# JasonTStanley/MultiDroneSim

Hardware: NVIDIA B200
Metric: drone-steps/sec (DYN_GND_DRAG_DW + LQR + order-3 CBF-QP, 8 drones/env) (higher is better)
Workload: dtype f32

## Files before the change

include/mds_b200.h:

```cpp
#ifndef MDS_B200_H
#define MDS_B200_H

#ifdef __cplusplus
extern "C" {
#endif

#define MDS_ABI_VERSION 9
#define MDS_MAX_DRONES_PER_ENV 32
#define MDS_MAX_OBSTACLES 8
#define MDS_OBS_DIM 20
#define MDS_REF_DIM 11

#define MDS_OK 0
#define MDS_ERR_ARG (-1)
#define MDS_ERR_LAUNCH (-2)
#define MDS_ERR_UNSUPPORTED (-3)

enum { MDS_DRONE_CF2X = 0, MDS_DRONE_CF2P = 1 };
enum { MDS_PHYSICS_DYN = 0, MDS_PHYSICS_DYN_GND_DRAG_DW = 1 };

enum { MDS_QP_OPTIMAL = 0, MDS_QP_INFEASIBLE = 1, MDS_QP_ITER_CAP = 2 };

enum {
  MDS_CTRL_GEOMETRIC = 0,
// ... 69 lines not shown
  int max_iter;
  int no_state_bounds;
} MdsCbfParams;

typedef struct MdsTrajSpecF32 { int kind, seg_begin, seg_count, pad; float p[8]; } MdsTrajSpecF32;
typedef struct MdsTrajSpecF64 { int kind, seg_begin, seg_count, pad; double p[8]; } MdsTrajSpecF64;
typedef struct MdsTrajSegF32 { int kind; int has_rot; float t_end; float dur; float p[24]; float rot[12]; } MdsTrajSegF32;
typedef struct MdsTrajSegF64 { int kind; int has_rot; double t_end; double dur; double p[24]; double rot[12]; } MdsTrajSegF64;

enum {
  MDS_STAT_DRONE_STEPS = 0, MDS_STAT_SUM_POS_ERR = 1, MDS_STAT_MAX_POS_ERR = 2,
  MDS_STAT_MIN_BARRIER = 3, MDS_STAT_QP_SOLVES = 4, MDS_STAT_QP_ITERS = 5,
  MDS_STAT_QP_INFEASIBLE = 6, MDS_STAT_QP_ITER_CAP = 7, MDS_STAT_COUNT = 8
};

typedef struct MdsRolloutCfg {
  int ctrl;
  int use_cbf;
  int num_obstacles;
  int write_obs_every;
  int stages;
  double obstacles[MDS_MAX_OBSTACLES * 4];
  const void* lqr_gain_planes_dev;
} MdsRolloutCfg;

int mds_abi_version(void);
const char* mds_last_error(void);
int mds_device_info(int* sm_count, int* cc_major, int* cc_minor, int* l2_bytes);

#include <stddef.h>
int mds_device_alloc(size_t bytes, void** out_dev);
int mds_device_free(void* dev);
int mds_copy_to_device(void* dst_dev, const void* src_host, size_t bytes, void* stream);
int mds_copy_to_host(void* dst_host, const void* src_dev, size_t bytes, void* stream);
int mds_stream_synchronize(void* stream);

int mds_physics_step_f32(const MdsDroneParams* prm, MdsState st, const float* action_dev,
                         const float* ext_force_dev, float* obs_dev, int E, int N, void* stream);
int mds_physics_step_f64(const MdsDroneParams* prm, MdsState st, const double* action_dev,
                         const double* ext_force_dev, double* obs_dev, int E, int N, void* stream);
int mds_physics_step_host_f32(const MdsDroneParams* prm, MdsState st, const float* action_host, float* action_dev,
                              float* obs_dev, float* obs_host, int E, int N, void* stream);
int mds_physics_step_host_f64(const MdsDroneParams* prm, MdsState st, const double* action_host, double* action_dev,
                              double* obs_dev, double* obs_host, int E, int N, void* stream);
int mds_obs_from_state_f32(const MdsDroneParams* prm, MdsState st, float* obs_dev, int D, void* stream);
int mds_obs_from_state_f64(const MdsDroneParams* prm, MdsState st, double* obs_dev, int D, void* stream);
// ... 97 lines not shown
```

multidronesim_b200/_lib.py:

```python
from __future__ import annotations

import ctypes as C
import os

_HERE = os.path.dirname(os.path.abspath(__file__))
LIB_PATH = os.environ.get("MDS_B200_LIB") or os.path.join(_HERE, "csrc", "libmds_b200.so")

MAX_DRONES_PER_ENV = 32
MAX_OBSTACLES = 8
OBS_DIM = 20
REF_DIM = 11
STAT_COUNT = 8
STAT_NAMES = ("drone_steps", "sum_pos_err", "max_pos_err", "min_barrier",
              "qp_solves", "qp_iters", "qp_infeasible", "qp_iter_cap")

DRONE_CF2X, DRONE_CF2P = 0, 1
PHYSICS_DYN, PHYSICS_DYN_GND_DRAG_DW = 0, 1
QP_OPTIMAL, QP_INFEASIBLE, QP_ITER_CAP = 0, 1, 2
CTRL_GEOMETRIC, CTRL_LQR_TORQUE, CTRL_LQR_OMEGA, CTRL_LQR_YANK, CTRL_DSLPID = 0, 1, 2, 3, 4
TRAJ_WAIT, TRAJ_CIRCLE, TRAJ_LEMNISCATE, TRAJ_TABLE = 0, 1, 2, 3
SEG_WAIT, SEG_CIRCLE, SEG_LEMNISCATE, SEG_LINE = 0, 1, 2, 3


class MdsError(RuntimeError):
# ... 28 lines not shown

class GeoGains(C.Structure):
    _fields_ = [(n, C.c_double) for n in ("kp", "kv", "kr", "kw", "g_ctrl", "max_tilt")]


class LqrGains(C.Structure):
    _fields_ = [("K", C.c_double * 48), ("dim", C.c_int)]


class CbfParams(C.Structure):
    _fields_ = [("order", C.c_int), ("zscale", C.c_double), ("safety_radius", C.c_double),
                ("kcbf", C.c_double * 3), ("umax", C.c_double * 4), ("fmin", C.c_double),
                ("fmax", C.c_double), ("max_iter", C.c_int), ("no_state_bounds", C.c_int)]


class RlsCfg(C.Structure):
    _fields_ = [("m", C.c_int), ("target", C.c_int), ("predict_from_xtp1", C.c_int), ("normalize_gain", C.c_int),
                ("project", C.c_int), ("drones_per_env", C.c_int), ("dt", C.c_double), ("theta_code", C.c_ubyte * (16 * 12))]


class RolloutCfg(C.Structure):
    _fields_ = [("ctrl", C.c_int), ("use_cbf", C.c_int), ("num_obstacles", C.c_int),
                ("write_obs_every", C.c_int), ("stages", C.c_int), ("obstacles", C.c_double * (MAX_OBSTACLES * 4)),
                ("lqr_gain_planes_dev", C.c_void_p)]


def traj_spec_dtype(real):
    import numpy as np
    return np.dtype([("kind", "i4"), ("seg_begin", "i4"), ("seg_count", "i4"), ("pad", "i4"), ("p", real, (8,))], align=True)


def traj_seg_dtype(real):
    import numpy as np
    return np.dtype([("kind", "i4"), ("has_rot", "i4"), ("t_end", real), ("dur", real),
                     ("p", real, (24,)), ("rot", real, (12,))], align=True)


_P = C.c_void_p
_I = C.c_int
_D = C.c_double
_PRM = C.POINTER(DroneParams)

_SIGS = {
    "mds_physics_step": [_PRM, State, _P, _P, _P, _I, _I, _P],
    "mds_physics_step_host": [_PRM, State, _P, _P, _P, _P, _I, _I, _P],
    "mds_obs_from_state": [_PRM, State, _P, _I, _P],
    "mds_traj_eval": [_P, _P, _D, _P, _I, _P],
# ... 114 lines not shown
```

multidronesim_b200/csrc/mds_kernels.cu:

```cuda
#include <cuda_runtime.h>
#include <stdio.h>
#include <stdlib.h>
#include <string.h>

#include <mutex>

#include "mds_cbf.cuh"
#include "mds_common.cuh"
#include "mds_ctrl.cuh"
#include "mds_physics.cuh"
#include "mds_sysid.cuh"
#include "mds_traj.cuh"

using namespace mds;

static thread_local char g_err[512] = "";
static int fail(int code, const char* fmt, const char* a = "") {
  snprintf(g_err, sizeof(g_err), fmt, a);
  return code;
}
static int check_launch(const char* what) {
  cudaError_t e = cudaGetLastError();
  if (e != cudaSuccess) {
    snprintf(g_err, sizeof(g_err), "%s: %s", what, cudaGetErrorString(e));
// ... 652 lines not shown
    MDS_REQUIRE(!cfg->use_cbf, "rollout: the CBF filter needs an LQR_OMEGA / LQR_YANK nominal controller");
    Dg = to_dev<Real>(*dsl);
  } else {
    MDS_REQUIRE(lqr && lqr_dim_ok(cfg->ctrl, lqr->dim), "rollout: LQR gains missing or of the wrong dimension");
    L = to_dev<Real>(*lqr);
    if (cfg->ctrl != MDS_CTRL_LQR_TORQUE) MDS_REQUIRE(pid.a && pid.b, "rollout: PID state missing");
  }
  if (cfg->use_cbf) {
    int rc = cbf_args_ok(cbf, N, cfg->num_obstacles);
    if (rc) return rc;
    MDS_REQUIRE((cfg->ctrl == MDS_CTRL_LQR_OMEGA && cbf->order == 2) || (cfg->ctrl == MDS_CTRL_LQR_YANK && cbf->order == 3),
                "rollout: CBF order 2 needs LQR_OMEGA, order 3 needs LQR_YANK");
    C = to_dev<Real>(*cbf);
    rc = qp_scratch_for(N, &C.scr);
    if (rc) return rc;
    for (int i = 0; i < cfg->num_obstacles * 4; ++i) R.obstacles[i] = Real(cfg->obstacles[i]);
    R.u0_pre = Real(prm->m * prm->g);
    R.u0_post = cbf->order == 2 ? Real(prm->m * prm->g) : Real(0);
  } else {
    R.n_obs = 0;
  }
  MDS_REQUIRE(!(cfg->write_obs_every > 0) || obs_log, "rollout: obs_log buffer missing");
  MDS_REQUIRE(cfg->write_obs_every <= 32767, "rollout: write_obs_every must be <= 32767");
  const int NP = next_pow2(N), threads = R.use_cbf ? cbf_block_threads<Real>(NP, N, R.n_obs) : MDS_BLOCK, epb = threads / NP;
  const int blocks = (E + epb - 1) / epb;
  size_t smem = R.use_cbf ? cbf_smem_bytes<Real>(threads, NP, N, R.n_obs) : 32;
  cudaStream_t cs = (cudaStream_t)stream;
  const DroneP<Real> Pd = to_dev<Real>(*prm);
  const StateP<Real> Sd = to_dev<Real>(st);
  const PidP<Real> Pi = to_dev<Real>(pid);
  const size_t obs_elems = (size_t)E * N * MDS_OBS_DIM;
  int mode = cfg->stages == 0 ? mds_rollout_plan(E, N) : cfg->stages;
  if (mode == 7 && cfg->stages == 0 && (cfg->ctrl == MDS_CTRL_DSLPID || NP > 32)) mode = 6;
  MDS_REQUIRE(!(mode == 7 && (cfg->ctrl == MDS_CTRL_DSLPID || NP > 32)), "rollout: plan 7 does not take the DSL PID controller");
  auto obs_slot = [&](int j) -> Real* {
    if (R.write_obs_every > 0 && (j % R.write_obs_every) == 0) return obs_log + (size_t)(j / R.write_obs_every - 1) * obs_elems;
    return obs;
  };
  cudaError_t attr_err = cudaSuccess;
  RolloutLaunch<Real> RL{Pd, R, G, L, C, Dg, Ds, Sd, Pi, specs, segs, action, fext, obs, obs_log, stats, E, N, NP, blocks, threads, phys_spec_of(*prm), smem, cs};
  auto keep = [&](cudaError_t e) { if (e != cudaSuccess) attr_err = e; };
  auto launch_loop = [&]() {
    RolloutLaunch<Real> RLL = RL;
    RLL.threads = R.use_cbf ? cbf_block_threads<Real>(NP, N, R.n_obs, loop_block<Real>()) : loop_block<Real>();
    if (const char* force = getenv("MDS_LOOP_THREADS")) { const int t = atoi(force); if (t >= 32 && t <= RLL.threads && t % 32 == 0) RLL.threads = t; }
    if (RLL.threads < NP) RLL.threads = NP;
    const int epb_l = RLL.threads / NP;
    RLL.blocks = (E + epb_l - 1) / epb_l;
    RLL.smem = R.use_cbf ? cbf_smem_bytes<Real>(RLL.threads, NP, N, R.n_obs) : 32;
    const int every = R.write_obs_every;
    int chunk = 16384;
    if (every > 0) chunk = every >= 16384 ? every : (16384 / every) * every;
    for (int k0 = 0; k0 < K; k0 += chunk) {
      RolloutLaunch<Real> part = RLL;
      if (every > 0) part.obs_log = obs_log + (size_t)(k0 / every) * obs_elems;
      keep(launch_loop_kernel<Real>(part, t0 + k0 * prm->dt_ctrl, prm->dt_ctrl, K - k0 < chunk ? K - k0 : chunk));
    }
  };
  cudaError_t queue_err = cudaSuccess;
  auto launch_queue = [&]() {
    RolloutLaunch<Real> RLQ = RL;
    RLQ.threads = R.use_cbf ? cbf_block_threads<Real>(NP, N, R.n_obs, loop_block<Real>()) : loop_block<Real>();
    if (RLQ.threads < 32) RLQ.threads = 32;
// ... 242 lines not shown
```

multidronesim_b200/csrc/mds_rollout.cuh:

```cuda
#pragma once
#include <cuda_runtime.h>
#include "mds_cbf.cuh"
#include "mds_common.cuh"
#include "mds_ctrl.cuh"
#include "mds_physics.cuh"
#include "mds_traj.cuh"

using namespace mds;

#ifndef MDS_BLOCK
#define MDS_BLOCK 256
#endif
#ifndef MDS_CTRL_MINB
#define MDS_CTRL_MINB 4
#endif
#ifndef MDS_LOOP_MINB
#define MDS_LOOP_MINB 2
#endif
#ifndef MDS_LOOP_BLOCK
#define MDS_LOOP_BLOCK 256
#endif
#ifndef MDS_LOOP_BLOCK_F64
#define MDS_LOOP_BLOCK_F64 192
#endif
// ... 428 lines not shown
  Real obstacles[MDS_MAX_OBSTACLES * 4];
  const Real* lqr_planes;
  int lqr_D;
};

MDS_DEV void atomic_min_double(double* addr, double v) {
  v += 0.0;
  if (v >= 0.0) atomicMin(reinterpret_cast<long long*>(addr), __double_as_longlong(v));
  else atomicMax(reinterpret_cast<unsigned long long*>(addr), (unsigned long long)__double_as_longlong(v));
}
MDS_DEV void atomic_max_double(double* addr, double v) {
  v += 0.0;
  if (v >= 0.0) atomicMax(reinterpret_cast<long long*>(addr), __double_as_longlong(v));
  else atomicMin(reinterpret_cast<unsigned long long*>(addr), (unsigned long long)__double_as_longlong(v));
}

MDS_DEV void prefetch_l1(const void* p) { asm volatile("prefetch.global.L1 [%0];" ::"l"(p)); }

struct StepStats {
  float err, min_h;
  int qp_solves, qp_iters, qp_infeas, qp_cap;
};

template <typename Real, int CTRL, bool USE_CBF, bool PDK = false, int SPEC = 0, int NT = 0>
MDS_DEV void ctrl_body(const DroneP<Real>& P, const RolloutP<Real>& Rc, const GeoP<Real>& G, const LqrP<Real>& L, const CbfP<Real>& C,
                       const DslP<Real>& Dg, const DslStateP<Real>& dst, const CbfSmem<Real>& S, const PidP<Real>& pid,
                       const typename TrajSpecT<Real>::spec& spec,
                       const typename TrajSpecT<Real>::seg* __restrict__ segs, const Obs<Real>& o, const GroupMap& g, int N, int NP,
                       double t, Real rpm[4], StepStats& ss, int pid_idx, M3<Real>* R_out = nullptr) {
  constexpr bool HAS_PID = (CTRL == MDS_CTRL_LQR_OMEGA || CTRL == MDS_CTRL_LQR_YANK);
  constexpr int ORD = CTRL == MDS_CTRL_LQR_OMEGA ? 2 : 3;
  Real u[4] = {Real(0), Real(0), Real(0), Real(0)};
  Ref<Real> ref;
  if (g.valid) {
    ref = eval_traj<Real>(spec, segs, t);
    ss.err = (float)norm(o.p - ref.p);
    if (CTRL == MDS_CTRL_GEOMETRIC) {
      geometric_input(P, G, o, ref, u);
      input_to_action<SPEC>(P, u, rpm);
    } else if (CTRL == MDS_CTRL_DSLPID) {
      DslState<Real> ds = load_dsl(dst, g.d);
      V3<Real> pe;
      dslpid_control(P, Dg, ds, o, ref.p, v3(Real(0), Real(0), ref.yaw), ref.v, v3(Real(0), Real(0), ref.yaw_rate), rpm, &pe);
      store_dsl(dst, g.d, ds);
    } else {
      if (PDK) dlqr_input(P, Rc.lqr_planes, (size_t)Rc.lqr_D, (size_t)g.d, CTRL, o, ref, u);
      else lqr_input(P, L, CTRL, o, ref, u);
      if (CTRL == MDS_CTRL_LQR_TORQUE) input_to_action<SPEC>(P, u, rpm);
    }
  }
  if (HAS_PID) {
    if (USE_CBF) {
      CbfAgent<Real> ag;
      ag.p = {Real(0), Real(0), Real(0)}; ag.dv = ag.p; ag.da = ag.p;
      Real F = Real(0), unom[4] = {Real(0), Real(0), Real(0), Real(0)}, usafe[4] = {Real(0), Real(0), Real(0), Real(0)};
      if (g.valid) {
        if (CTRL == MDS_CTRL_LQR_OMEGA) u[0] = cap_thrust(P, u[0]);
        Real xd[10];
// ... 129 lines not shown
  __shared__ typename Vec4T<Real>::type sm_pos[MDS_BLOCK];
  const int N = ct_n<NT>(N_rt), NP = ct_np<NT>(NP_rt);
  CbfSmem<Real> S = cbf_smem_carve<Real>(smem_raw, NP, N, Rc.n_obs);
  GroupMap g = group_map(N, NP, E);
  StepStats ss = {0.f, 1e30f, 0, 0, 0, 0};
  if (g.env_valid) {
    full_group_hint<NT>(g);
    if (g.valid) {
      prefetch_l1(specs + g.d);
      prefetch_l1(reinterpret_cast<const char*>(specs + g.d) + 32);
      if (CTRL == MDS_CTRL_LQR_OMEGA || CTRL == MDS_CTRL_LQR_YANK) { prefetch_l1(pid.a + g.d); prefetch_l1(pid.b + g.d); }
    }
    const Obs<Real> o = physics_body(P, st, action, fext, obs_out, sm_pos + (threadIdx.x - g.n), g, N, NP);
    Real rpm[4] = {Real(0), Real(0), Real(0), Real(0)};
    typename TrajSpecT<Real>::spec spec;
    spec.kind = MDS_TRAJ_WAIT;
    if (g.valid) spec = specs[g.d];
    ctrl_body<Real, CTRL, USE_CBF>(P, Rc, G, L, C, Dg, dst, S, pid, spec, segs, o, g, N, NP, t, rpm, ss, g.d);
    if (g.valid) store4(action, g.d, rpm);
  }
  if (stats) stats_block_reduce<USE_CBF>(stats, g.valid ? 1 : 0, ss, ss.err);
}

template <typename Real, int CTRL, bool USE_CBF, int NT, int SPEC>
__global__ void __launch_bounds__(loop_block<Real>(), MDS_LOOP_MINB) rollout_loop_kernel(DroneP<Real> P, RolloutP<Real> Rc, GeoP<Real> G, LqrP<Real> L, CbfP<Real> C,
                                                                  DslP<Real> Dg, DslStateP<Real> dst, StateP<Real> st, PidP<Real> pid,
                                                                  const typename TrajSpecT<Real>::spec* __restrict__ specs,
                                                                  const typename TrajSpecT<Real>::seg* __restrict__ segs,
                                                                  Real* __restrict__ action, const Real* __restrict__ fext, Real* __restrict__ obs,
                                                                  Real* __restrict__ obs_log, double* __restrict__ stats, double t0, double dt_ctrl, int K, int E,
                                                                  int N_rt, int NP_rt) {
  extern __shared__ __align__(32) unsigned char smem_raw[];
  using R4 = typename Vec4T<Real>::type;
  __shared__ R4 sm_pos[USE_CBF ? 1 : loop_block<Real>()];
  constexpr bool STAGE = sizeof(Real) == 4;
  __shared__ __align__(16) typename TrajSpecT<Real>::spec sm_spec[STAGE ? loop_block<Real>() : 1];
  constexpr bool HAS_PID = (CTRL == MDS_CTRL_LQR_OMEGA || CTRL == MDS_CTRL_LQR_YANK);
  __shared__ R4 sm_pid_a[(STAGE && HAS_PID) ? loop_block<Real>() : 1];
  __shared__ typename Vec2T<Real>::type sm_pid_b[(STAGE && HAS_PID) ? loop_block<Real>() : 1];
  const PidP<Real> pid_s = STAGE ? PidP<Real>{sm_pid_a, sm_pid_b} : pid;
  const int N = ct_n<NT>(N_rt), NP = ct_np<NT>(NP_rt);
  CbfSmem<Real> S = cbf_smem_carve<Real>(smem_raw, NP, N, Rc.n_obs);
  GroupMap g = group_map(N, NP, E);
  R4* const env_pos = USE_CBF ? reinterpret_cast<R4*>(S.env0 + (size_t)g.el * S.stride) : sm_pos + (threadIdx.x - g.n);
  StepStats acc = {0.f, 1e30f, 0, 0, 0, 0};
  float max_err = 0.f;
  int steps_done = 0;
#ifndef MDS_NO_FULLW
  constexpr bool FULLW = STAGE && HAS_PID && NT > 1 && NT < 32 && (NT & (NT - 1)) == 0;
#else
  constexpr bool FULLW = false;
#endif
  const bool live = g.env_valid;
  if (FULLW) {
    const int first_env = g.e - (int)((threadIdx.x & 31) / NP);
    g.env_valid = first_env < E;
    if (g.env_valid && !live) { g.e = E - 1; g.d = g.e * N + g.n; }
    g.cmask = 0xffffffffu;
  }
  if (g.env_valid) {
    full_group_hint<NT>(g);
    Obs<Real> o;
    V3<Real> wb = {Real(0), Real(0), Real(0)};
    typename TrajSpecT<Real>::spec spec_reg;
    typename TrajSpecT<Real>::spec& spec = STAGE ? sm_spec[threadIdx.x] : spec_reg;
    spec.kind = MDS_TRAJ_WAIT;
    V3<Real> fx_reg = {Real(0), Real(0), Real(0)};
    const bool has_fx = fext != nullptr;
    if (g.valid) {
      o = load_obs(obs, g.d);
      spec = specs[g.d];
      wb = {st.pos_wx[g.d].w, st.vel_wy[g.d].w, st.wz[g.d]};
      if (has_fx && !STAGE) fx_reg = {fext[3 * g.d], fext[3 * g.d + 1], fext[3 * g.d + 2]};
      if (STAGE && HAS_PID) { sm_pid_a[threadIdx.x] = pid.a[g.d]; sm_pid_b[threadIdx.x] = pid.b[g.d]; }
    }
    Real rpm[4] = {Real(0), Real(0), Real(0), Real(0)};
    const size_t obs_elems = (size_t)E * N * MDS_OBS_DIM;
    int log_countdown = Rc.write_obs_every;
    Real* log_slot = obs_log;
    for (int k = 0; k < K; ++k) {
      StepStats ss = {0.f, 1e30f, 0, 0, 0, 0};
      M3<Real> R;
      ctrl_body<Real, CTRL, USE_CBF, (NT < 0), SPEC, NT>(P, Rc, G, L, C, Dg, dst, S, pid_s, spec, segs, o, g, N, NP, t0 + (double)k * dt_ctrl, rpm, ss,
                                                     STAGE ? (int)threadIdx.x : g.d, HAS_PID ? &R : nullptr);
      acc.err += ss.err; max_err = fmaxf(max_err, ss.err); acc.min_h = fminf(acc.min_h, ss.min_h);
      acc.qp_solves += ss.qp_solves; acc.qp_iters += ss.qp_iters; acc.qp_infeas += ss.qp_infeas + (ss.qp_cap << 16);
      Drone<Real> s;
      s.p = o.p; s.qx = o.qx; s.qy = o.qy; s.qz = o.qz; s.qw = o.qw; s.v = o.v; s.w = wb;
#pragma unroll
      for (int i = 0; i < 4; ++i) s.rpm[i] = o.rpm[i];
      V3<Real> fx = fx_reg;
      if (STAGE) {
        fx = {Real(0), Real(0), Real(0)};
        if (has_fx && g.valid) fx = {__ldg(fext + 3 * g.d), __ldg(fext + 3 * g.d + 1), __ldg(fext + 3 * g.d + 2)};
      }
      o = physics_core<SPEC>(P, s, rpm, fx, env_pos, g, N, NP, HAS_PID ? &R : nullptr);
      wb = s.w;
      if (Rc.write_obs_every > 0 && --log_countdown == 0) {
        if (g.valid && live) store_obs(log_slot, g.d, o, true);
        log_slot += obs_elems;
        log_countdown = Rc.write_obs_every;
      }
    }
    if (g.valid && live) {
      Drone<Real> s;
      s.p = o.p; s.qx = o.qx; s.qy = o.qy; s.qz = o.qz; s.qw = o.qw; s.v = o.v; s.w = wb;
#pragma unroll
// ... 177 lines not shown
```

multidronesim_b200/csrc/mds_rollout_launch.cuh:

```cuda
#pragma once
#include <cuda_runtime.h>
#include "mds_rollout.cuh"

template <typename Real> struct RolloutLaunch {
  DroneP<Real> Pd;
  RolloutP<Real> R;
  GeoP<Real> G;
  LqrP<Real> L;
  CbfP<Real> C;
  DslP<Real> Dg;
  DslStateP<Real> Ds;
  StateP<Real> Sd;
  PidP<Real> Pi;
  const typename TrajSpecT<Real>::spec* specs;
  const typename TrajSpecT<Real>::seg* segs;
  Real* action;
  const Real* fext;
  Real* obs;
  Real* obs_log;
  double* stats;
  int E, N, NP, blocks, threads;
  int spec;
  size_t smem;
  cudaStream_t cs;
};

template <typename Real> cudaError_t launch_loop_kernel(const RolloutLaunch<Real>& a, double t0, double dt_ctrl, int K);
template <typename Real> cudaError_t launch_ctrl_kernel(const RolloutLaunch<Real>& a, double t, const Real* obs_in, bool set_attr);
template <typename Real> cudaError_t launch_fused_kernel(const RolloutLaunch<Real>& a, double t, Real* obs_out, bool set_attr);
template <typename Real> cudaError_t launch_queue_kernel(const RolloutLaunch<Real>& a, double t0, double dt_ctrl, int K, RolloutQueue q, int sm_count, bool query_only,
                                                         int* blocks_per_sm);
```

multidronesim_b200/csrc/mds_rollout_tu.cu:

```cuda
#include "mds_rollout_launch.cuh"

#ifndef MDS_TU_REAL
#error "compile with -DMDS_TU_REAL=float or double"
#endif
#ifndef MDS_TU_KIND
#error "compile with -DMDS_TU_KIND=0, 1, 2 or 3"
#endif
using Real = MDS_TU_REAL;

template <typename F> static void dispatch_ctrl(int ctrl, int use_cbf, F&& f) {
  switch (ctrl) {
    case MDS_CTRL_GEOMETRIC: f.template run<MDS_CTRL_GEOMETRIC, false, false>(); break;
    case MDS_CTRL_LQR_TORQUE: f.template run<MDS_CTRL_LQR_TORQUE, false, true>(); break;
    case MDS_CTRL_DSLPID: f.template run<MDS_CTRL_DSLPID, false, false>(); break;
    case MDS_CTRL_LQR_OMEGA:
      if (use_cbf) f.template run<MDS_CTRL_LQR_OMEGA, true, true>();
      else f.template run<MDS_CTRL_LQR_OMEGA, false, true>();
      break;
    default:
      if (use_cbf) f.template run<MDS_CTRL_LQR_YANK, true, true>();
      else f.template run<MDS_CTRL_LQR_YANK, false, true>();
      break;
  }
}

#if MDS_TU_KIND == 0
struct LoopLauncher {
  const RolloutLaunch<Real>& a;
  double t0, dt_ctrl;
  int K;
  cudaError_t err;
  template <int CT, bool CB, bool PDKC> void run() {
    const bool pdk = a.R.lqr_planes != nullptr;
    auto kern = pdk ? rollout_loop_kernel<Real, CT, CB, (PDKC ? -1 : 0), 0>
                    : (a.spec == 1 ? ((a.N == 8) ? rollout_loop_kernel<Real, CT, CB, 8, 1> : rollout_loop_kernel<Real, CT, CB, 0, 1>)
                                   : ((a.N == 8) ? rollout_loop_kernel<Real, CT, CB, 8, 0> : rollout_loop_kernel<Real, CT, CB, 0, 0>));
    err = cudaFuncSetAttribute(kern, cudaFuncAttributeMaxDynamicSharedMemorySize, (int)a.smem);
    kern<<<a.blocks, a.threads, a.smem, a.cs>>>(a.Pd, a.R, a.G, a.L, a.C, a.Dg, a.Ds, a.Sd, a.Pi, a.specs, a.segs, a.action, a.fext, a.obs, a.obs_log,
                                                 a.stats, t0, dt_ctrl, K, a.E, a.N, a.NP);
  }
};
template <> cudaError_t launch_loop_kernel<Real>(const RolloutLaunch<Real>& a, double t0, double dt_ctrl, int K) {
  LoopLauncher l{a, t0, dt_ctrl, K, cudaSuccess};
  dispatch_ctrl(a.R.ctrl, a.R.use_cbf, l);
  return l.err;
}
#elif MDS_TU_KIND == 1
struct CtrlLauncher {
  const RolloutLaunch<Real>& a;
  double t;
  const Real* obs_in;
  bool set_attr;
  cudaError_t err;
  template <int CT, bool CB, bool PDKC> void run() {
    const bool pdk = a.R.lqr_planes != nullptr;
    auto kern = pdk ? ctrl_step_kernel<Real, CT, CB, (PDKC ? -1 : 0)>
                    : ((a.N == 8) ? ctrl_step_kernel<Real, CT, CB, 8> : ctrl_step_kernel<Real, CT, CB, 0>);
    if (set_attr) err = cudaFuncSetAttribute(kern, cudaFuncAttributeMaxDynamicSharedMemorySize, (int)a.smem);
    int grid = a.blocks;
// ... 70 lines not shown
```

multidronesim_b200/csrc/mds_traj.cuh:

```cuda
#pragma once
#include "mds_common.cuh"

namespace mds {

template <typename Real> struct TrajSpecT;
template <> struct TrajSpecT<float> { using spec = MdsTrajSpecF32; using seg = MdsTrajSegF32; };
template <> struct TrajSpecT<double> { using spec = MdsTrajSpecF64; using seg = MdsTrajSegF64; };

template <typename Real> struct Ref {
  V3<Real> p, v, a;
  Real yaw, yaw_rate;
};

MDS_DEV double reduce_2pi(double th) {
  const double two_pi = 6.283185307179586476925286766559, inv_two_pi = 0.15915494309189533576888376337251;
  return th - two_pi * floor(th * inv_two_pi);
}

template <typename Real> MDS_DEV Ref<Real> eval_circle(const Real* p, double t) {
  const double pi = 3.14159265358979323846, two_pi = 2.0 * pi;
  Real r = p[0], v = p[1];
  double wt = (double)v / (double)r * t;
  Real s, c;
  sincos_(Real(reduce_2pi(wt)), &s, &c);
// ... 110 lines not shown
  double total = (double)segs[b + n - 1].t_end;
  if (t >= total) return eval_segment<Real>(segs[b + n - 1], (double)segs[b + n - 1].dur);
  int k = 0;
  double t0 = 0.0;
  while (k < n - 1 && t > (double)segs[b + k].t_end) {
    t0 = (double)segs[b + k].t_end;
    ++k;
  }
  return eval_segment<Real>(segs[b + k], t - t0);
}

template <typename Real>
MDS_DEV Ref<Real> eval_traj(const typename TrajSpecT<Real>::spec& sp, const typename TrajSpecT<Real>::seg* __restrict__ segs, double t) {
  switch (sp.kind) {
    case MDS_TRAJ_CIRCLE: return eval_circle<Real>(sp.p, t);
    case MDS_TRAJ_LEMNISCATE: return eval_lemniscate<Real>(sp.p, t);
    case MDS_TRAJ_WAIT: return eval_wait<Real>(sp.p);
    default: break;
  }
  const typename TrajSpecT<Real>::spec table_spec = sp;
  return eval_traj_table<Real>(table_spec, segs, t);
}

}
```

multidronesim_b200/rollout.py:

```python
from __future__ import annotations

import torch

from . import _lib
from .control.dslpid import DSLPIDControl
from .control.geometric import GeometricControl
from .control.lqr import LQRController, LQROmegaController, LQRYankOmegaController
from .control.dlqr import _DecentralizedBase


class FusedRollout:
    def __init__(self, env, trajs, controller, qp_tracker=None, obstacles=None):
        self.env, self.trajs, self.controller, self.qp = env, trajs, controller, qp_tracker
        if trajs.num != env.NUM_TOTAL:
            raise ValueError("need one trajectory per drone")
        cfg = _lib.RolloutCfg()
        if isinstance(controller, GeometricControl):
            cfg.ctrl = _lib.CTRL_GEOMETRIC
        elif isinstance(controller, DSLPIDControl):
            cfg.ctrl = _lib.CTRL_DSLPID
        elif isinstance(controller, _DecentralizedBase):
            if controller.K is None or controller._coupled:
                raise _lib.MdsError("FusedRollout takes a decentralised LQR with per-drone gains: call compute_controller() first "
                                    "(the robot-coupled 12-dim gain runs through PerCallPipeline)")
            cfg.ctrl = controller.VARIANT
        elif isinstance(controller, LQROmegaController):
            cfg.ctrl = _lib.CTRL_LQR_OMEGA
        elif isinstance(controller, LQRYankOmegaController):
            cfg.ctrl = _lib.CTRL_LQR_YANK
        elif isinstance(controller, LQRController):
            cfg.ctrl = _lib.CTRL_LQR_TORQUE
        else:
            raise TypeError("unsupported controller type")
        cfg.use_cbf = int(qp_tracker is not None)
        rows = [] if obstacles is None else (obstacles.tolist() if isinstance(obstacles, torch.Tensor) else list(obstacles))
        if len(rows) > _lib.MAX_OBSTACLES:
# ... 6 lines not shown
                cfg.obstacles[4 * i + k] = float(r[k])
        cfg.write_obs_every = 0
        self.cfg = cfg
        self.stats = torch.zeros(_lib.STAT_COUNT, device=env.device, dtype=torch.float64)
        self.reset_stats()
        self.t = 0.0

    def reset_stats(self):
        self.stats.zero_()
        self.stats[3] = 1e30

    def plan(self):
        return _lib.load_library().mds_rollout_plan(self.env.NUM_ENVS, self.env.NUM_DRONES)

    def run(self, K, t0=None, obs_log=None, log_every=0, stages=0):
        env = self.env
        if t0 is None:
            t0 = self.t
        if stages not in (0, 1, 2, 3, 4, 5, 6, 7):
            raise ValueError("stages must be 0..7")
        t_call = t0 + env.CTRL_TIMESTEP if stages == 5 else t0
        self.cfg.stages = int(stages)
        self.cfg.write_obs_every = int(log_every) if obs_log is not None else 0
        if obs_log is not None:
            _lib.require_cuda(obs_log, "obs_log", env.dtype)
            if obs_log.numel() < (K // max(1, log_every)) * env.NUM_TOTAL * _lib.OBS_DIM:
                raise ValueError("obs_log too small")
        is_lqr = self.cfg.ctrl in (_lib.CTRL_LQR_TORQUE, _lib.CTRL_LQR_OMEGA, _lib.CTRL_LQR_YANK)
        geo = self.controller.c_gains() if self.cfg.ctrl == _lib.CTRL_GEOMETRIC else None
        per_drone = isinstance(self.controller, _DecentralizedBase)
        if per_drone:
            if self.controller._coupled:
                raise _lib.MdsError("robot-coupled gains cannot run in the fused rollout")
            self.cfg.lqr_gain_planes_dev = self.controller.K_planes.data_ptr()
            lqr = _lib.LqrGains()
            lqr.dim = self.controller.m
            pid = self.controller.low_level.pid_struct() if self.controller.low_level is not None else _lib.PidState(None, None)
        else:
            self.cfg.lqr_gain_planes_dev = None
            lqr = self.controller.c_gains() if is_lqr else None
            pid = self.controller._pid() if is_lqr else _lib.PidState(None, None)
        dsl = self.controller.c_gains() if self.cfg.ctrl == _lib.CTRL_DSLPID else None
        dsl_state = self.controller.state_struct() if self.cfg.ctrl == _lib.CTRL_DSLPID else _lib.DslPidState(None, None, None)
        cbf = self.qp.cbf.c_params() if self.qp is not None else None
        _lib.call("mds_rollout", env.dtype, env._prm, self.cfg, geo, lqr, cbf, env._state_struct(), pid, dsl, dsl_state,
                  _lib.ptr(self.trajs.specs), _lib.ptr(self.trajs.segs), _lib.ptr(env._obs), _lib.ptr(env._action), _lib.ptr(env._ext_force), _lib.ptr(obs_log),
# ... 162 lines not shown
```

multidronesim_b200/scenarios.py:

```python
from __future__ import annotations

import math

import numpy as np
import torch

from . import _lib
from .cbf import DroneCBF, DroneQPTracker
from .control import (GeometricControl, LQROmegaController, LQRYankOmegaController, ThrustOmegaController,
                      YankOmegaController)
from .enums import DroneModel, Physics
from .envs import BatchedCtrlAviary
from .model import LinearizedOmegaModel, LinearizedYankOmegaModel
from .rollout import FusedRollout
from .trajectories import TrajectorySet


SWARM_OBSTACLES = [[0.2, 0.0, 0.5, 0.1]]


def lemniscate_pos(a, theta, center):
    s, c = np.sin(theta), np.cos(theta)
    den = 1 + s * s
    return np.stack([center[0] + a * s * c / den, center[1] + a * c / den, np.full_like(theta, center[2])], axis=-1)
# ... 25 lines not shown
    return init


def cbf_swarm(num_envs, num_drones=8, order=3, dtype=torch.float32, device="cuda", seed=3, env_offset=0,
              omega=0.5, obstacle=True, physics=Physics.DYN_GND_DRAG_DW, pyb_freq=240, ctrl_freq=240):
    E, N = int(num_envs), int(num_drones)
    center = np.array([0.0, 0.0, 0.5])
    phase = (2 * np.pi / (N + 0.25)) * np.arange(N)
    init = cbf_swarm_init(E, N, seed=seed, env_offset=env_offset)
    env = BatchedCtrlAviary(drone_model=DroneModel.CF2P, num_drones=N, initial_xyzs=init, physics=physics,
                            pyb_freq=pyb_freq, ctrl_freq=ctrl_freq, num_envs=E, device=device, dtype=dtype)
    if order == 3:
        mdl = LinearizedYankOmegaModel(env)
        ctrl = LQRYankOmegaController(env, mdl, YankOmegaController(env))
        cbf = DroneCBF(env, [mdl] * N, safety_radius=0.125, zscale=2, order=3, cbf_poles=np.array([-3.0, -3.6, -5.6]))
        trk = DroneQPTracker(cbf, order=3, num_robots=N, xdim=10, env=env)
    else:
        mdl = LinearizedOmegaModel(env)
        ctrl = LQROmegaController(env, mdl, ThrustOmegaController(env))
        cbf = DroneCBF(env, [mdl] * N, safety_radius=0.1, zscale=1, order=2, cbf_poles=np.array([-2.2, -2.4]))
        trk = DroneQPTracker(cbf, order=2, num_robots=N, xdim=9, env=env)
    params = np.zeros((N, 7))
    params[:, 0], params[:, 1], params[:, 2:5], params[:, 5], params[:, 6] = 1.0, omega, center, 0.0, phase
    trajs = TrajectorySet.from_arrays(_lib.TRAJ_LEMNISCATE, np.tile(params, (E, 1)), device=device, dtype=dtype)
    obstacles = [list(o) for o in SWARM_OBSTACLES] if obstacle else None
    rollout = FusedRollout(env, trajs, ctrl, trk, obstacles)
    return dict(env=env, ctrl=ctrl, cbf=cbf, tracker=trk, trajs=trajs, obstacles=obstacles, rollout=rollout, init=init)


def cbf_swarm_streams(num_envs, parts, num_drones=8, order=3, dtype=torch.float32, device="cuda", seed=3, env_offset=0, **kw):
    from .dist import env_shard
    from .rollout import SwarmStreams
    subs = []
    for p in range(int(parts)):
        b0, b1 = env_shard(int(num_envs), p, int(parts))
        subs.append(cbf_swarm(b1 - b0, num_drones, order=order, dtype=dtype, device=device, seed=seed, env_offset=env_offset + b0, **kw))
    return SwarmStreams([s["rollout"] for s in subs]), subs


def tracking_swarm(num_envs, dtype=torch.float32, device="cuda", seed=1, env_offset=0, physics=Physics.DYN_GND_DRAG_DW):
    E = int(num_envs)
    ids = env_offset + np.arange(E)
    kind = np.where(ids % 2 == 0, _lib.TRAJ_CIRCLE, _lib.TRAJ_LEMNISCATE)
    phase = 2 * np.pi * 0.5 * (1.0 + np.vectorize(math.erf)(counter_normal(seed + 1000, ids, 1)[:, 0] / math.sqrt(2.0)))
    params = np.zeros((E, 7))
    circ = kind == _lib.TRAJ_CIRCLE
    params[circ, 0:6] = [1.0, 0.5, 0.0, 0.0, 1.0, 0.0]
# ... 11 lines not shown
```

multidronesim_b200/trajectories/__init__.py:

```python
from __future__ import annotations

import math

import numpy as np
import torch

from .. import _lib


class TrajectoryBase:
    def get_total_time(self):
        raise NotImplementedError

    def segments(self):
        raise NotImplementedError

    def simple_spec(self):
        return None


class CircleTrajectory(TrajectoryBase):
    def __init__(self, r=1.0, v=.5, center=np.array([0, 0, 0]), yaw_rate=0, revolutions=None, duration=None):
        self.r, self.v, self.yaw_rate = float(r), float(v), float(yaw_rate)
        self.center = np.asarray(center, dtype=float)
# ... 143 lines not shown
        for d, tr in enumerate(trajs):
            simple = tr.simple_spec()
            if simple is not None:
                kind, p = simple
                specs[d]["kind"] = kind
                specs[d]["p"][:len(p)] = p
            else:
                sg = tr.segments()
                specs[d]["kind"] = _lib.TRAJ_TABLE
                specs[d]["seg_begin"], specs[d]["seg_count"] = len(segs), len(sg)
                specs[d]["pad"] = 0 if isinstance(tr, CompoundTrajectory) else 1
                t_end = 0.0
                for kind, dur, p, rot in sg:
                    t_end += dur
                    segs.append((kind, rot is not None, t_end, dur, p, rot))
        seg_arr = np.zeros(max(1, len(segs)), dtype=_lib.traj_seg_dtype(real))
        for k, (kind, has_rot, t_end, dur, p, rot) in enumerate(segs):
            seg_arr[k]["kind"], seg_arr[k]["has_rot"], seg_arr[k]["t_end"], seg_arr[k]["dur"] = kind, int(has_rot), t_end, dur
            seg_arr[k]["p"][:len(p)] = p
            if rot is not None:
                seg_arr[k]["rot"][:] = rot
        if num_envs > 1:
            specs = np.tile(specs, num_envs)
        self._finish(specs, seg_arr)

    def _finish(self, specs, seg_arr):
        self.num = len(specs)
        self.specs = torch.from_numpy(specs.view(np.uint8).copy()).to(self.device)
        self.segs = torch.from_numpy(seg_arr.view(np.uint8).copy()).to(self.device)
        self.ref = torch.zeros(self.num, _lib.REF_DIM, device=self.device, dtype=self.dtype)

    @classmethod
    def from_arrays(cls, kind, params, device="cuda", dtype=torch.float32):
        self = cls.__new__(cls)
        _lib.load_library()
        self.device, self.dtype = torch.device(device), dtype
        real = "f4" if dtype == torch.float32 else "f8"
        params = np.asarray(params, dtype=float)
        specs = np.zeros(params.shape[0], dtype=_lib.traj_spec_dtype(real))
        specs["kind"] = kind
        specs["p"][:, :params.shape[1]] = params
        self._finish(specs, np.zeros(1, dtype=_lib.traj_seg_dtype(real)))
        return self

    def eval(self, t, out=None):
        out = self.ref if out is None else out
        _lib.call("mds_traj_eval", self.dtype, _lib.ptr(self.specs), _lib.ptr(self.segs), float(t), _lib.ptr(out),
                  self.num, _lib.stream_ptr(self.device))
        return out

    def __call__(self, t):
        r = self.eval(t)
        return r[:, 0:3], r[:, 3:6], r[:, 6:9], r[:, 9], r[:, 10]
```

Measured before the change: 20.74 billion.

## Share per-block trajectory reference table across envs with identical trajectories

When every environment uses the same per-drone trajectory specs, the rollout kernel builds a shared-memory table of reference states for the next 32 control steps, indexed by drone slot. Each thread then reads its reference from that table instead of evaluating the trajectory itself. This cuts the redundant per-thread trajectory evaluation, mostly trigonometry, and the per-thread spec staging. The price is block-wide syncs every 32 steps, extra shared memory, and an env_period detection step on the host that only covers the f32, N=8, LQR-omega/yank path.

```diff
diff --git a/include/mds_b200.h b/include/mds_b200.h
--- a/include/mds_b200.h
+++ b/include/mds_b200.h
@@ -115,6 +115,7 @@
   int stages;
   double obstacles[MDS_MAX_OBSTACLES * 4];
   const void* lqr_gain_planes_dev;
+  int traj_period;
 } MdsRolloutCfg;
 
 int mds_abi_version(void);
diff --git a/multidronesim_b200/_lib.py b/multidronesim_b200/_lib.py
--- a/multidronesim_b200/_lib.py
+++ b/multidronesim_b200/_lib.py
@@ -74,7 +74,7 @@
 class RolloutCfg(C.Structure):
     _fields_ = [("ctrl", C.c_int), ("use_cbf", C.c_int), ("num_obstacles", C.c_int),
                 ("write_obs_every", C.c_int), ("stages", C.c_int), ("obstacles", C.c_double * (MAX_OBSTACLES * 4)),
-                ("lqr_gain_planes_dev", C.c_void_p)]
+                ("lqr_gain_planes_dev", C.c_void_p), ("traj_period", C.c_int)]
 
 
 def traj_spec_dtype(real):
diff --git a/multidronesim_b200/csrc/mds_kernels.cu b/multidronesim_b200/csrc/mds_kernels.cu
--- a/multidronesim_b200/csrc/mds_kernels.cu
+++ b/multidronesim_b200/csrc/mds_kernels.cu
@@ -698,6 +698,7 @@
   }
   MDS_REQUIRE(!(cfg->write_obs_every > 0) || obs_log, "rollout: obs_log buffer missing");
   MDS_REQUIRE(cfg->write_obs_every <= 32767, "rollout: write_obs_every must be <= 32767");
+  MDS_REQUIRE(cfg->traj_period == 0 || cfg->traj_period == N, "rollout: traj_period must be 0 or the drone count N");
   const int NP = next_pow2(N), threads = R.use_cbf ? cbf_block_threads<Real>(NP, N, R.n_obs) : MDS_BLOCK, epb = threads / NP;
   const int blocks = (E + epb - 1) / epb;
   size_t smem = R.use_cbf ? cbf_smem_bytes<Real>(threads, NP, N, R.n_obs) : 32;
@@ -714,7 +715,8 @@
     return obs;
   };
   cudaError_t attr_err = cudaSuccess;
-  RolloutLaunch<Real> RL{Pd, R, G, L, C, Dg, Ds, Sd, Pi, specs, segs, action, fext, obs, obs_log, stats, E, N, NP, blocks, threads, phys_spec_of(*prm), smem, cs};
+  RolloutLaunch<Real> RL{Pd, R, G, L, C, Dg, Ds, Sd, Pi, specs, segs, action, fext, obs, obs_log, stats, E, N, NP, blocks, threads, phys_spec_of(*prm), smem, cs,
+                         cfg->traj_period};
   auto keep = [&](cudaError_t e) { if (e != cudaSuccess) attr_err = e; };
   auto launch_loop = [&]() {
     RolloutLaunch<Real> RLL = RL;
diff --git a/multidronesim_b200/csrc/mds_rollout.cuh b/multidronesim_b200/csrc/mds_rollout.cuh
--- a/multidronesim_b200/csrc/mds_rollout.cuh
+++ b/multidronesim_b200/csrc/mds_rollout.cuh
@@ -474,18 +474,20 @@
   int qp_solves, qp_iters, qp_infeas, qp_cap;
 };
 
-template <typename Real, int CTRL, bool USE_CBF, bool PDK = false, int SPEC = 0, int NT = 0>
+template <typename Real, int CTRL, bool USE_CBF, bool PDK = false, int SPEC = 0, int NT = 0, bool REFTAB = false>
 MDS_DEV void ctrl_body(const DroneP<Real>& P, const RolloutP<Real>& Rc, const GeoP<Real>& G, const LqrP<Real>& L, const CbfP<Real>& C,
                        const DslP<Real>& Dg, const DslStateP<Real>& dst, const CbfSmem<Real>& S, const PidP<Real>& pid,
                        const typename TrajSpecT<Real>::spec& spec,
                        const typename TrajSpecT<Real>::seg* __restrict__ segs, const Obs<Real>& o, const GroupMap& g, int N, int NP,
-                       double t, Real rpm[4], StepStats& ss, int pid_idx, M3<Real>* R_out = nullptr) {
+                       double t, Real rpm[4], StepStats& ss, int pid_idx, M3<Real>* R_out = nullptr,
+                       const typename Vec4T<Real>::type* ref_slot = nullptr) {
   constexpr bool HAS_PID = (CTRL == MDS_CTRL_LQR_OMEGA || CTRL == MDS_CTRL_LQR_YANK);
   constexpr int ORD = CTRL == MDS_CTRL_LQR_OMEGA ? 2 : 3;
   Real u[4] = {Real(0), Real(0), Real(0), Real(0)};
   Ref<Real> ref;
   if (g.valid) {
-    ref = eval_traj<Real>(spec, segs, t);
+    if constexpr (REFTAB) ref = load_ref<Real>(ref_slot);
+    else ref = eval_traj<Real>(spec, segs, t);
     ss.err = (float)norm(o.p - ref.p);
     if (CTRL == MDS_CTRL_GEOMETRIC) {
       geometric_input(P, G, o, ref, u);
@@ -661,7 +663,20 @@
   if (stats) stats_block_reduce<USE_CBF>(stats, g.valid ? 1 : 0, ss, ss.err);
 }
 
-template <typename Real, int CTRL, bool USE_CBF, int NT, int SPEC>
+#ifndef MDS_REF_STEPS
+#define MDS_REF_STEPS 32
+#endif
+template <typename Real, int NT>
+__device__ __noinline__ void build_ref_table(typename Vec4T<Real>::type* tab, const typename TrajSpecT<Real>::spec* __restrict__ specs,
+                                             const typename TrajSpecT<Real>::seg* __restrict__ segs, double t0, double dt_ctrl, int k0, int steps) {
+  for (int i = threadIdx.x; i < steps * NT; i += blockDim.x) {
+    const int j = i / NT, n = i - j * NT;
+    const typename TrajSpecT<Real>::spec sp = specs[n];
+    store_ref<Real>(tab + 3 * i, eval_traj<Real>(sp, segs, t0 + (double)(k0 + j) * dt_ctrl));
+  }
+}
+
+template <typename Real, int CTRL, bool USE_CBF, int NT, int SPEC, bool REFTAB = false>
 __global__ void __launch_bounds__(loop_block<Real>(), MDS_LOOP_MINB) rollout_loop_kernel(DroneP<Real> P, RolloutP<Real> Rc, GeoP<Real> G, LqrP<Real> L, CbfP<Real> C,
                                                                   DslP<Real> Dg, DslStateP<Real> dst, StateP<Real> st, PidP<Real> pid,
                                                                   const typename TrajSpecT<Real>::spec* __restrict__ specs,
@@ -673,7 +688,8 @@
   using R4 = typename Vec4T<Real>::type;
   __shared__ R4 sm_pos[USE_CBF ? 1 : loop_block<Real>()];
   constexpr bool STAGE = sizeof(Real) == 4;
-  __shared__ __align__(16) typename TrajSpecT<Real>::spec sm_spec[STAGE ? loop_block<Real>() : 1];
+  __shared__ __align__(16) typename TrajSpecT<Real>::spec sm_spec[(STAGE && !REFTAB) ? loop_block<Real>() : 1];
+  __shared__ R4 sm_ref[REFTAB ? 3 * MDS_REF_STEPS * NT : 1];
   constexpr bool HAS_PID = (CTRL == MDS_CTRL_LQR_OMEGA || CTRL == MDS_CTRL_LQR_YANK);
   __shared__ R4 sm_pid_a[(STAGE && HAS_PID) ? loop_block<Real>() : 1];
   __shared__ typename Vec2T<Real>::type sm_pid_b[(STAGE && HAS_PID) ? loop_block<Real>() : 1];
@@ -690,10 +706,12 @@
 #else
   constexpr bool FULLW = false;
 #endif
+  static_assert(!REFTAB || (FULLW && NT * MDS_REF_STEPS <= 8 * 32 && (MDS_REF_STEPS & (MDS_REF_STEPS - 1)) == 0),
+                "the reference table needs the full-warp instantiation and at most 12 KB of shared memory");
   const bool live = g.env_valid;
   if (FULLW) {
     const int first_env = g.e - (int)((threadIdx.x & 31) / NP);
-    g.env_valid = first_env < E;
+    g.env_valid = REFTAB || first_env < E;
     if (g.env_valid && !live) { g.e = E - 1; g.d = g.e * N + g.n; }
     g.cmask = 0xffffffffu;
   }
@@ -702,26 +720,39 @@
     Obs<Real> o;
     V3<Real> wb = {Real(0), Real(0), Real(0)};
     typename TrajSpecT<Real>::spec spec_reg;
-    typename TrajSpecT<Real>::spec& spec = STAGE ? sm_spec[threadIdx.x] : spec_reg;
+    typename TrajSpecT<Real>::spec& spec = (STAGE && !REFTAB) ? sm_spec[threadIdx.x] : spec_reg;
     spec.kind = MDS_TRAJ_WAIT;
     V3<Real> fx_reg = {Real(0), Real(0), Real(0)};
     const bool has_fx = fext != nullptr;
     if (g.valid) {
       o = load_obs(obs, g.d);
-      spec = specs[g.d];
+      if (!REFTAB) spec = specs[g.d];
       wb = {st.pos_wx[g.d].w, st.vel_wy[g.d].w, st.wz[g.d]};
       if (has_fx && !STAGE) fx_reg = {fext[3 * g.d], fext[3 * g.d + 1], fext[3 * g.d + 2]};
       if (STAGE && HAS_PID) { sm_pid_a[threadIdx.x] = pid.a[g.d]; sm_pid_b[threadIdx.x] = pid.b[g.d]; }
+    }
+    if constexpr (REFTAB) {
+      build_ref_table<Real, NT>(sm_ref, specs, segs, t0, dt_ctrl, 0, min(K, MDS_REF_STEPS));
+      __syncthreads();
     }
     Real rpm[4] = {Real(0), Real(0), Real(0), Real(0)};
     const size_t obs_elems = (size_t)E * N * MDS_OBS_DIM;
     int log_countdown = Rc.write_obs_every;
     Real* log_slot = obs_log;
     for (int k = 0; k < K; ++k) {
+      const int row = k & (MDS_REF_STEPS - 1);
+      if constexpr (REFTAB) {
+        if (k > 0 && row == 0) {
+          __syncthreads();
+          build_ref_table<Real, NT>(sm_ref, specs, segs, t0, dt_ctrl, k, min(K - k, MDS_REF_STEPS));
+          __syncthreads();
+        }
+      }
       StepStats ss = {0.f, 1e30f, 0, 0, 0, 0};
       M3<Real> R;
-      ctrl_body<Real, CTRL, USE_CBF, (NT < 0), SPEC, NT>(P, Rc, G, L, C, Dg, dst, S, pid_s, spec, segs, o, g, N, NP, t0 + (double)k * dt_ctrl, rpm, ss,
-                                                     STAGE ? (int)threadIdx.x : g.d, HAS_PID ? &R : nullptr);
+      ctrl_body<Real, CTRL, USE_CBF, (NT < 0), SPEC, NT, REFTAB>(P, Rc, G, L, C, Dg, dst, S, pid_s, spec, segs, o, g, N, NP, t0 + (double)k * dt_ctrl,
+                                                             rpm, ss, STAGE ? (int)threadIdx.x : g.d, HAS_PID ? &R : nullptr,
+                                                             REFTAB ? sm_ref + 3 * (row * NT + g.n) : nullptr);
       acc.err += ss.err; max_err = fmaxf(max_err, ss.err); acc.min_h = fminf(acc.min_h, ss.min_h);
       acc.qp_solves += ss.qp_solves; acc.qp_iters += ss.qp_iters; acc.qp_infeas += ss.qp_infeas + (ss.qp_cap << 16);
       Drone<Real> s;
diff --git a/multidronesim_b200/csrc/mds_rollout_launch.cuh b/multidronesim_b200/csrc/mds_rollout_launch.cuh
--- a/multidronesim_b200/csrc/mds_rollout_launch.cuh
+++ b/multidronesim_b200/csrc/mds_rollout_launch.cuh
@@ -23,6 +23,7 @@
   int spec;
   size_t smem;
   cudaStream_t cs;
+  int traj_period;
 };
 
 template <typename Real> cudaError_t launch_loop_kernel(const RolloutLaunch<Real>& a, double t0, double dt_ctrl, int K);
diff --git a/multidronesim_b200/csrc/mds_rollout_tu.cu b/multidronesim_b200/csrc/mds_rollout_tu.cu
--- a/multidronesim_b200/csrc/mds_rollout_tu.cu
+++ b/multidronesim_b200/csrc/mds_rollout_tu.cu
@@ -35,6 +35,10 @@
     auto kern = pdk ? rollout_loop_kernel<Real, CT, CB, (PDKC ? -1 : 0), 0>
                     : (a.spec == 1 ? ((a.N == 8) ? rollout_loop_kernel<Real, CT, CB, 8, 1> : rollout_loop_kernel<Real, CT, CB, 0, 1>)
                                    : ((a.N == 8) ? rollout_loop_kernel<Real, CT, CB, 8, 0> : rollout_loop_kernel<Real, CT, CB, 0, 0>));
+    if constexpr (sizeof(Real) == 4 && (CT == MDS_CTRL_LQR_OMEGA || CT == MDS_CTRL_LQR_YANK)) {
+      if (!pdk && a.N == 8 && a.traj_period == 8)
+        kern = a.spec == 1 ? rollout_loop_kernel<Real, CT, CB, 8, 1, true> : rollout_loop_kernel<Real, CT, CB, 8, 0, true>;
+    }
     err = cudaFuncSetAttribute(kern, cudaFuncAttributeMaxDynamicSharedMemorySize, (int)a.smem);
     kern<<<a.blocks, a.threads, a.smem, a.cs>>>(a.Pd, a.R, a.G, a.L, a.C, a.Dg, a.Ds, a.Sd, a.Pi, a.specs, a.segs, a.action, a.fext, a.obs, a.obs_log,
                                                  a.stats, t0, dt_ctrl, K, a.E, a.N, a.NP);
diff --git a/multidronesim_b200/csrc/mds_traj.cuh b/multidronesim_b200/csrc/mds_traj.cuh
--- a/multidronesim_b200/csrc/mds_traj.cuh
+++ b/multidronesim_b200/csrc/mds_traj.cuh
@@ -156,4 +156,19 @@
   return eval_traj_table<Real>(table_spec, segs, t);
 }
 
+template <typename Real> MDS_DEV void store_ref(typename Vec4T<Real>::type* w, const Ref<Real>& r) {
+  typename Vec4T<Real>::type w0, w1, w2;
+  w0.x = r.p.x; w0.y = r.p.y; w0.z = r.p.z; w0.w = r.v.x;
+  w1.x = r.v.y; w1.y = r.v.z; w1.z = r.a.x; w1.w = r.a.y;
+  w2.x = r.a.z; w2.y = r.yaw; w2.z = r.yaw_rate; w2.w = Real(0);
+  w[0] = w0; w[1] = w1; w[2] = w2;
 }
+template <typename Real> MDS_DEV Ref<Real> load_ref(const typename Vec4T<Real>::type* w) {
+  const typename Vec4T<Real>::type w0 = w[0], w1 = w[1], w2 = w[2];
+  Ref<Real> r;
+  r.p = {w0.x, w0.y, w0.z}; r.v = {w0.w, w1.x, w1.y}; r.a = {w1.z, w1.w, w2.x};
+  r.yaw = w2.y; r.yaw_rate = w2.z;
+  return r;
+}
+
+}
diff --git a/multidronesim_b200/rollout.py b/multidronesim_b200/rollout.py
--- a/multidronesim_b200/rollout.py
+++ b/multidronesim_b200/rollout.py
@@ -10,8 +10,9 @@
 
 
 class FusedRollout:
-    def __init__(self, env, trajs, controller, qp_tracker=None, obstacles=None):
+    def __init__(self, env, trajs, controller, qp_tracker=None, obstacles=None, ref_table=True):
         self.env, self.trajs, self.controller, self.qp = env, trajs, controller, qp_tracker
+        self.ref_table = ref_table
         if trajs.num != env.NUM_TOTAL:
             raise ValueError("need one trajectory per drone")
         cfg = _lib.RolloutCfg()
@@ -64,6 +65,8 @@
         t_call = t0 + env.CTRL_TIMESTEP if stages == 5 else t0
         self.cfg.stages = int(stages)
         self.cfg.write_obs_every = int(log_every) if obs_log is not None else 0
+        N = env.NUM_DRONES
+        self.cfg.traj_period = N if (self.ref_table and self.trajs.env_period == N) else 0
         if obs_log is not None:
             _lib.require_cuda(obs_log, "obs_log", env.dtype)
             if obs_log.numel() < (K // max(1, log_every)) * env.NUM_TOTAL * _lib.OBS_DIM:
diff --git a/multidronesim_b200/scenarios.py b/multidronesim_b200/scenarios.py
--- a/multidronesim_b200/scenarios.py
+++ b/multidronesim_b200/scenarios.py
@@ -71,7 +71,7 @@
         trk = DroneQPTracker(cbf, order=2, num_robots=N, xdim=9, env=env)
     params = np.zeros((N, 7))
     params[:, 0], params[:, 1], params[:, 2:5], params[:, 5], params[:, 6] = 1.0, omega, center, 0.0, phase
-    trajs = TrajectorySet.from_arrays(_lib.TRAJ_LEMNISCATE, np.tile(params, (E, 1)), device=device, dtype=dtype)
+    trajs = TrajectorySet.from_arrays(_lib.TRAJ_LEMNISCATE, np.tile(params, (E, 1)), device=device, dtype=dtype, drones_per_env=N)
     obstacles = [list(o) for o in SWARM_OBSTACLES] if obstacle else None
     rollout = FusedRollout(env, trajs, ctrl, trk, obstacles)
     return dict(env=env, ctrl=ctrl, cbf=cbf, tracker=trk, trajs=trajs, obstacles=obstacles, rollout=rollout, init=init)
diff --git a/multidronesim_b200/trajectories/__init__.py b/multidronesim_b200/trajectories/__init__.py
--- a/multidronesim_b200/trajectories/__init__.py
+++ b/multidronesim_b200/trajectories/__init__.py
@@ -189,16 +189,26 @@
                 seg_arr[k]["rot"][:] = rot
         if num_envs > 1:
             specs = np.tile(specs, num_envs)
-        self._finish(specs, seg_arr)
-
-    def _finish(self, specs, seg_arr):
+        self._finish(specs, seg_arr, n_unique)
+
+    def _finish(self, specs, seg_arr, env_period):
         self.num = len(specs)
         self.specs = torch.from_numpy(specs.view(np.uint8).copy()).to(self.device)
         self.segs = torch.from_numpy(seg_arr.view(np.uint8).copy()).to(self.device)
         self.ref = torch.zeros(self.num, _lib.REF_DIM, device=self.device, dtype=self.dtype)
+        self.env_period = env_period
+
+    @property
+    def specs(self):
+        return self._specs
+
+    @specs.setter
+    def specs(self, value):
+        self._specs = value
+        self.env_period = 0
 
     @classmethod
-    def from_arrays(cls, kind, params, device="cuda", dtype=torch.float32):
+    def from_arrays(cls, kind, params, device="cuda", dtype=torch.float32, drones_per_env=None):
         self = cls.__new__(cls)
         _lib.load_library()
         self.device, self.dtype = torch.device(device), dtype
@@ -207,7 +217,11 @@
         specs = np.zeros(params.shape[0], dtype=_lib.traj_spec_dtype(real))
         specs["kind"] = kind
         specs["p"][:, :params.shape[1]] = params
-        self._finish(specs, np.zeros(1, dtype=_lib.traj_seg_dtype(real)))
+        period = 0
+        if drones_per_env and len(specs) % int(drones_per_env) == 0:
+            envs = specs.view(np.uint8).reshape(len(specs) // int(drones_per_env), -1)
+            period = int(drones_per_env) if bool((envs == envs[0]).all()) else 0
+        self._finish(specs, np.zeros(1, dtype=_lib.traj_seg_dtype(real)), period)
         return self
 
     def eval(self, t, out=None):
```

Measured after the change: 22.99 billion (median of 6 runs). 10.9% higher.
